# jean-pierreBoth/kmerutils

Measured on AMD Instinct MI355X. Metric: Gbases/sec k-mer+sketch throughput, k=31, 200 sketches/read, higher is better.
Workload: dtype u64; 1 GPU; ont_k31: 746333 ONT-shaped reads (log-normal lengths, 8% errors), 4.38e+09 bases, k=31, ProbMinHash3a m=200 + kmercount 8-bit; workload_name=ont_k31, reads_per_gpu=746333, bases_per_gpu=4379626696, kmers_per_gpu=4357236706, k=31, sketch_size=200, sketch=True, count=True, parallelism=reads sharded x1

## Files before the change

kmerutils_amd/csrc/kmu_pmh_points.hip:

```cpp
#include "kmu_pmh_steps.h"

namespace kmu {

static constexpr uint32_t PTS_REFRESH_MASK = 15u;

template <bool UNIT_W = false>
__device__ __forceinline__ bool pmh3a_first_point_may_matter(const SketchArgs &a, bool sig32, uint64_t qb, uint64_t key,
                                                             uint32_t w, const double *winv_lut, uint64_t &s0, uint64_t &s3) {
    const uint64_t seed = hasher_finish(KMU_HASHER_NOHASH, key, sig32);
    s0 = splitmix_at(seed, 1);
    s3 = splitmix_at(seed, 4);
    const uint64_t r1 = rotl64(s0 + s3, 23) + s0;
    const double u1 = __longlong_as_double((long long) ((r1 >> 12) | 0x3FF0000000000000ull)) - 1.0;
    const double x = a.e01.c1 * u1;
    if (UNIT_W) return !(x < 1.0) || x < __longlong_as_double((long long) qb);
    return !(x < 1.0) || winv_of(winv_lut, w) * x < __longlong_as_double((long long) qb);
}

__device__ __forceinline__ void pmh3a_first_point_rest(const SketchArgs &a, bool sig32, uint64_t *hmin, uint64_t *sig,
                                                       const uint64_t *qmax_sh, bool have, uint64_t key, uint32_t w,
                                                       uint64_t s0, uint64_t s3, const double *winv_lut) {
    const uint64_t qb = __hip_atomic_load(qmax_sh, __ATOMIC_RELAXED, __HIP_MEMORY_SCOPE_WORKGROUP);
    if (have) {
        const double winv = winv_of(winv_lut, w);
        const uint64_t r1 = rotl64(s0 + s3, 23) + s0;
        const double u1 = __longlong_as_double((long long) ((r1 >> 12) | 0x3FF0000000000000ull)) - 1.0;
        double x = a.e01.c1 * u1;
        const double qmax = __longlong_as_double((long long) qb);
        const bool slow = !(x < 1.0);
        if (slow || winv * x < qmax) {
            const uint64_t seed = hasher_finish(KMU_HASHER_NOHASH, key, sig32);
            Xoshiro rng;
            rng.s0 = s0;
            rng.s3 = s3;
            rng.s1 = splitmix_at(seed, 2);
            rng.s2 = splitmix_at(seed, 3);
            (void) rng.next();
            if (slow) x = exp01_rest(a.e01, rng);
            const double h = winv * x;
            if (h < qmax) slot_update_wave(hmin, sig, draw_slot(a, rng), h, key);
        }
    }
}

__global__ void __launch_bounds__(256) k_pts_long_list(const uint32_t *lst_n, uint32_t n_seq, uint32_t thr, uint32_t *out) {
    const uint32_t r = blockIdx.x * blockDim.x + threadIdx.x;
    if (r < n_seq && lst_n[r] > thr) out[2 + atomicAdd(&out[0], 1u)] = r;
}
__device__ __forceinline__ uint64_t wg4_qmax(const uint64_t *arrays, size_t wave_words, int m) {
    uint64_t q = 0;
    for (int t = lane_id(); t < m; t += 64) {
        uint64_t v = H_INIT;
#pragma unroll
        for (int w4 = 0; w4 < 4; w4++) {
            const uint64_t x = __hip_atomic_load(&arrays[(size_t) w4 * wave_words + t], __ATOMIC_RELAXED, __HIP_MEMORY_SCOPE_WORKGROUP);
            v = x < v ? x : v;
        }
        q = v > q ? v : q;
    }
    return wave_max_u64(q);
}

template <bool SIG32, bool WG>
__device__ __forceinline__ void pts_one_read(const SketchArgs &a, uint32_t r, uint8_t *smem, size_t wave_words, const double *winv_lut) {
    const int wave = threadIdx.x >> 6, lane = lane_id();
    constexpr bool sig32 = SIG32;
    constexpr uint32_t cstride = WG ? 256u : 64u;
    const uint32_t cstart = WG ? 64u * (uint32_t) wave : 0u;
    uint64_t *arrays = reinterpret_cast<uint64_t *>(smem);
    uint64_t *hmin = arrays + (size_t) wave * wave_words;
    uint64_t *sig = hmin + a.m;
    uint64_t *qmax_sh = sig + a.m;
    uint64_t *qk = qmax_sh + 2;
    uint32_t *qw = reinterpret_cast<uint32_t *>(qk + 128);
    uint64_t *qs0 = qk + 128 + 64, *qs3 = qs0 + 128;
    const uint64_t base = a.offsets[r] - a.offsets[0];
    const uint32_t n = uniform_u32(a.lst_n[r]);
    const uint32_t n_u = uniform_u32(a.lst_nu[r]);
    uint64_t tau_b = H_INIT;
    if (n >= a.tau_min_n) {
        const uint64_t len = a.offsets[r + 1] - a.offsets[r];
        const uint64_t kk = (uint64_t) a.cfg.k;
        const double tau = a.tau_num / (double) (len >= kk ? len - kk + 1 : 0);
        if (tau < 1.0) tau_b = (uint64_t) __double_as_longlong(tau);
        tau_b = uniform_u64(tau_b);
    }
    uint32_t wmax = 0;
    uint64_t qb = H_INIT;
    for (int turn = 0; turn < 2; turn++) {
        for (int t = lane; t < a.m; t += 64) { hmin[t] = H_INIT; sig[t] = 0; }
        if (lane == 0) *qmax_sh = tau_b;
        if (WG) __syncthreads();
        uint32_t chunk = 0, qn = 0;
        qb = tau_b;
        uint64_t key_nx = 0;
        uint32_t w_nx = 1;
        {
            const uint32_t i = cstart + (uint32_t) lane;
            if (i < n) { key_nx = a.lst_keys[base + i]; w_nx = i < n_u ? 1u : a.lst_w[base + i]; }
        }
        for (uint32_t c = cstart; c < n; c += cstride, chunk++) {
            const uint32_t i = c + (uint32_t) lane;
            const uint64_t key = key_nx;
            const uint32_t w = w_nx;
            const bool have = i < n && w != 0u;
            if (have) wmax = w > wmax ? w : wmax;
            if (i + cstride < n) key_nx = a.lst_keys[base + i + cstride];
            w_nx = 1u;
            if (c + cstride + 64u > n_u) {
                if (i + cstride < n && i + cstride >= n_u) w_nx = a.lst_w[base + i + cstride];
            }
            if ((chunk & (WG && chunk < 64u ? PTS_REFRESH_MASK >> 2 : PTS_REFRESH_MASK)) == 0u) {
                qb = WG ? wg4_qmax(arrays, wave_words, a.m) : wave_qmax(hmin, a.m);
                qb = qb < tau_b ? qb : tau_b;
                if (lane == 0) *qmax_sh = qb;
            }
            uint64_t s0 = 0, s3 = 0;
            const bool pass = c + 64u <= n_u ? have && pmh3a_first_point_may_matter<true>(a, sig32, qb, key, w, winv_lut, s0, s3)
                                             : have && pmh3a_first_point_may_matter(a, sig32, qb, key, w, winv_lut, s0, s3);
            const uint64_t pm = __ballot(pass);
            if (pass) {
                const uint32_t pos = qn + (uint32_t) __popcll(pm & ((1ull << lane) - 1ull));
                qk[pos] = key;
                qw[pos] = w;
                qs0[pos] = s0;
                qs3[pos] = s3;
            }
            qn += (uint32_t) __popcll(pm);
            if (qn >= 64u) {
                qn -= 64u;
                pmh3a_first_point_rest(a, sig32, hmin, sig, qmax_sh, true, qk[qn + lane], qw[qn + lane], qs0[qn + lane], qs3[qn + lane],
                                       winv_lut);
            }
        }
        if (qn) {
            const bool have = (uint32_t) lane < qn;
            pmh3a_first_point_rest(a, sig32, hmin, sig, qmax_sh, have, have ? qk[lane] : 0ull, have ? qw[lane] : 1u, have ? qs0[lane] : 0ull,
                                   have ? qs3[lane] : 0ull, winv_lut);
        }
        if (WG) {
            __syncthreads();
            qb = wg4_qmax(arrays, wave_words, a.m);
        } else qb = wave_qmax(hmin, a.m);
        if (tau_b == H_INIT || qb < tau_b) break;
        tau_b = H_INIT;
        if (lane == 0 && (!WG || wave == 0)) atomicAdd(a.tau_redo, 1u);
        if (WG) __syncthreads();
    }
    wmax = (uint32_t) wave_max_u64((uint64_t) wmax);
    if (n && wmax && winv_of(winv_lut, wmax) < __longlong_as_double((long long) qb)) {
        const uint32_t c0 = 1.0 < __longlong_as_double((long long) qb) ? 0u : (n_u & ~63u);
        uint32_t c = cstart;
        if (c < c0) c += (c0 - c + cstride - 1u) / cstride * cstride;
        for (; c < n; c += cstride) {
            const uint32_t i = c + (uint32_t) lane;
            double winv = 0.0;
            bool alive = false;
            if (i < n) {
                const uint32_t w = i < n_u ? 1u : a.lst_w[base + i];
                winv = winv_of(winv_lut, w);
                alive = w != 0u && winv < __longlong_as_double((long long) qb);
            }
            if (__any(alive)) pmh3a_more_points<true>(a, sig32, hmin, sig, qb, alive, alive ? a.lst_keys[base + i] : 0ull, winv);
        }
    }
    if (WG) {
        __syncthreads();
        for (int t = threadIdx.x; t < a.m; t += 256) {
            uint64_t bh = arrays[t], bk = arrays[a.m + t];
#pragma unroll
            for (int w4 = 1; w4 < 4; w4++) {
// ... 77 lines not shown
```

kmerutils_amd/csrc/kmu_api.hip:

```cpp
#include <algorithm>

#include "kmu_ctx.hpp"
#include "kmu_stream.h"

namespace kmu {

thread_local std::string g_create_error;

int check_kmer(kmu_ctx *ctx, int t, int k) {
    if (k <= 0) return fail(ctx, KMU_E_BAD_K, "kmer_size %d must be positive", k);
    int maxk = 0;
    switch (t) {
    case KMU_KMER32BIT: maxk = 14; break;
    case KMU_KMER16B32BIT:
        if (k != 16) return fail(ctx, KMU_E_BAD_K, "Kmer16b32bit has 16 bases, got %d", k);
        return KMU_OK;
    case KMU_KMER64BIT: maxk = 31; break;
    case KMU_KMERAA32BIT: maxk = 6; break;
    case KMU_KMERAA64BIT: maxk = 12; break;
    default: return fail(ctx, KMU_E_BAD_ARG, "unknown kmer_type %d", t);
    }
    if (k > maxk)
        return fail(ctx, KMU_E_BAD_K, "KmerSeqIterator cannot support so many bases for given kmer type, kmer size %d", k);
    return KMU_OK;
// ... 333 lines not shown
    KMU_HIP(ctx, hipStreamSynchronize(ctx->stream));
    KMU_HIP(ctx, hipHostFree(p));
    return KMU_OK;
}

int kmu_copy_to_device(kmu_ctx *ctx, void *dst_device, const void *src_host, uint64_t bytes) {
    if (!ctx || (bytes && (!dst_device || !src_host))) return KMU_E_BAD_ARG;
    KMU_HIP(ctx, hipSetDevice(ctx->device));
    KMU_HIP(ctx, hipMemcpyAsync(dst_device, src_host, bytes, hipMemcpyHostToDevice, ctx->stream));
    KMU_HIP(ctx, hipStreamSynchronize(ctx->stream));
    return KMU_OK;
}

int kmu_copy_to_host(kmu_ctx *ctx, void *dst_host, const void *src_device, uint64_t bytes) {
    if (!ctx || (bytes && (!dst_host || !src_device))) return KMU_E_BAD_ARG;
    KMU_HIP(ctx, hipSetDevice(ctx->device));
    KMU_HIP(ctx, hipMemcpyAsync(dst_host, src_device, bytes, hipMemcpyDeviceToHost, ctx->stream));
    KMU_HIP(ctx, hipStreamSynchronize(ctx->stream));
    return KMU_OK;
}

int kmu_profile_enable(kmu_ctx *ctx, int on) {
    if (!ctx) return KMU_E_BAD_ARG;
    if (!on && ctx->profiling) profile_collect(ctx);
    ctx->profiling = on != 0;
    return KMU_OK;
}
int kmu_profile_reset(kmu_ctx *ctx) {
    if (!ctx) return KMU_E_BAD_ARG;
    profile_collect(ctx);
    ctx->stats.clear();
    auto tr = ctx->bufs.find("pmh.tau_redo");
    if (tr != ctx->bufs.end() && tr->second.p) KMU_HIP(ctx, hipMemsetAsync(tr->second.p, 0, 4, ctx->stream));
    return KMU_OK;
}
int kmu_profile_get(kmu_ctx *ctx, kmu_kernel_stat *stats, int cap) {
    if (!ctx) return KMU_E_BAD_ARG;
    profile_collect(ctx);
    int n = 0;
    for (auto &kv : ctx->stats) {
        if (stats && n < cap) {
            memset(&stats[n], 0, sizeof(kmu_kernel_stat));
            strncpy(stats[n].name, kv.first.c_str(), sizeof(stats[n].name) - 1);
            stats[n].launches = kv.second.launches;
            stats[n].total_ms = kv.second.ms;
        }
        n++;
    }
    auto tr = ctx->bufs.find("pmh.tau_redo");
    if (tr != ctx->bufs.end() && tr->second.p) {
        uint32_t redone = 0;
        KMU_HIP(ctx, hipMemcpyAsync(&redone, tr->second.p, 4, hipMemcpyDeviceToHost, ctx->stream));
        KMU_HIP(ctx, hipStreamSynchronize(ctx->stream));
        if (redone) {
            if (stats && n < cap) {
                memset(&stats[n], 0, sizeof(kmu_kernel_stat));
                strncpy(stats[n].name, "pmh_tau_redone_reads", sizeof(stats[n].name) - 1);
                stats[n].launches = redone;
            }
            n++;
        }
    }
    return n;
}

int kmu_count_non_acgt(kmu_ctx *ctx, const uint8_t *bases, const uint64_t *offsets, uint32_t n_seq, int mem,
                       uint64_t *counts_out) {
    if (!ctx || !counts_out) return KMU_E_BAD_ARG;
    KMU_HIP(ctx, hipSetDevice(ctx->device));
    DevSeqs ds;
    KMU_TRY(stage_sequences(ctx, bases, offsets, nullptr, n_seq, KMU_INPUT_ASCII, mem, &ds));
    uint64_t *d_counts = counts_out;
    if (mem == KMU_MEM_HOST) {
        void *p;
        KMU_TRY(dev_buf(ctx, "out.u64", (size_t) n_seq * 8 + 8, &p));
        d_counts = (uint64_t *) p;
    }
    if (n_seq) {
        int grid = (int) std::min<uint32_t>(n_seq, (uint32_t) ctx->num_cus * 8);
        KernelTimer t(ctx, "k_count_non_acgt");
        hipLaunchKernelGGL(k_count_non_acgt, dim3(grid), dim3(256), 0, ctx->stream, ds.bases, ds.offsets, n_seq,
                           ds.total_bytes, d_counts);
    }
    KMU_HIP(ctx, hipGetLastError());
    if (mem == KMU_MEM_HOST)
        KMU_HIP(ctx, hipMemcpyAsync(counts_out, d_counts, (size_t) n_seq * 8, hipMemcpyDeviceToHost, ctx->stream));
    return finish_call(ctx, mem);
}

int kmu_pack2b(kmu_ctx *ctx, const uint8_t *bases, const uint64_t *offsets, uint32_t n_seq, int mem,
               uint8_t *packed_out, uint64_t *packed_offsets_out) {
// ... 100 lines not shown
```

kmerutils_amd/csrc/kmu_sketch_kernels.h:

```cpp
#pragma once

#include "kmu_ctx.hpp"
#include "kmu_device.h"

namespace kmu {

struct SketchArgs {
    const uint8_t *bases;
    const uint64_t *offsets;
    const uint64_t *packed_offsets;
    const uint64_t *block_rows;
    uint32_t n_seq;
    int packed;
    uint64_t total_bytes;
    KmerCfg cfg;
    int m;
    int hasher;
    int rand08;
    int sig_bytes;
    uint32_t block_size;
    uint32_t cap;
    uint32_t part_target;
    double inv_part_target;
    uint32_t tile_shift;
    uint64_t *scr_keys;
    uint32_t *scr_info;
    uint32_t *scr_w;
    uint32_t skip_longer;
    uint64_t *def_keys;
    int bk_shift;
    uint32_t bk_mask;
    uint32_t *tau_redo;
    double tau_num;
    uint32_t *counts_out;
    const void *hashed;
    int hashed_bytes;
// ... 13 lines not shown
    uint32_t idx_thresh;
    uint64_t idx_zone;
    uint32_t tau_min_n;
    Exp01 e01;
    void *sig_out;
    uint32_t *queue;
    uint32_t *err;
};

enum { M_READ = 0, M_NSCR = 1, M_NEXT = 2, M_DEF = 3, M_QMAX = 4 , M_FLAGS = 6 , M_WORDS = 8 };
static constexpr uint32_t DEF_CAP = 1u << 20;
static constexpr uint32_t DEF_PARTS = 32;
static constexpr uint32_t DEF_SEG = DEF_CAP / DEF_PARTS;
static constexpr uint32_t LONG_SEQ_KMERS = 1u << 18;
static constexpr int BUCKET_BITS = 12;
static constexpr uint32_t NBUCKETS = 1u << BUCKET_BITS;
static constexpr int QCHUNK = 4;
static constexpr int KREG = 10;
static constexpr uint32_t WINV_LUT = 256;
static constexpr size_t PTS_WAVE_WORDS = 2 + 128 + 64 + 256;
static constexpr double PTS_TAU_C = 4.6;
static constexpr int UQ_KREG = 20;
static constexpr uint32_t UQ1_BM = 17, UQ1_COLL = 1024, UQ2_BM = 18, UQ2_COLL = 2048;
template <int UQ_THREADS, uint32_t UQ_BM_BITS, uint32_t UQ_COLL>
struct UqShape {
    static constexpr uint32_t KEYS = (uint32_t) UQ_THREADS * UQ_KREG;
    static constexpr uint32_t BM_WORDS = (1u << UQ_BM_BITS) / 32;
    static constexpr uint32_t BUCKETS = 2u * UQ_THREADS;
    static constexpr uint32_t TILE = (KEYS + 32 + 15) / 16 + 3;
    static constexpr uint32_t RAW_WAVES = (TILE + 63) / 64;
    static constexpr size_t LDS = (size_t) BM_WORDS * 8 + (size_t) UQ_COLL * 20 + ((size_t) BUCKETS + 1 + TILE + UQ_THREADS / 64 + 8 + 8) * 4 + 64 +
                                  (size_t) RAW_WAVES * 1024 + 16;
};
static constexpr uint32_t SHORT_KEYS = 256, SHORT_SLOTS = 512, SHORT_WORDS = 24;
static constexpr size_t SHORT_WAVE_BYTES = (size_t) SHORT_SLOTS * 12 + SHORT_WORDS * 4;
static constexpr uint32_t SMALLK_WORDS = 32768;
static constexpr uint32_t SMALLK_TILE = 1024;

template <bool AA, bool BOTTOMK, bool EMIT = false, bool PLAIN = false>
__global__ void __launch_bounds__(1024) k_sketch_pmh3a(SketchArgs a);
__global__ void k_pts_long_list(const uint32_t *lst_n, uint32_t n_seq, uint32_t thr, uint32_t *out);
template <bool SIG32>
__global__ void __launch_bounds__(256) k_pmh_points(SketchArgs a);
template <int UQ_THREADS, uint32_t UQ_BM_BITS, uint32_t UQ_COLL, int MINW>
__global__ void __launch_bounds__(UQ_THREADS, MINW) k_multiset_uq(SketchArgs a);
__global__ void k_multiset_short(SketchArgs a);
template <bool SIG32>
__global__ void __launch_bounds__(256) k_pmh_points_short(SketchArgs a);
template <bool EMIT>
__global__ void __launch_bounds__(1024) k_sketch_smallk(SketchArgs a);
__global__ void k_pmh_reduce(const uint64_t *part_h, const uint64_t *part_k, uint64_t n_parts, int m, uint64_t stride, int sig_bytes, void *sig_out,
                             uint64_t *part_out);
__global__ void k_max_len(const uint64_t *offsets, uint32_t n_seq, uint64_t *out);
__global__ void k_nk_scan(const uint64_t *offsets, uint32_t n_seq, int k, uint64_t *koff, uint32_t *err);
__global__ void k_seq_hashes_compact(const uint8_t *bases, const uint64_t *offsets, const uint64_t *packed_offsets, uint32_t n_seq, int packed,
                                     uint64_t total, KmerCfg cfg, const uint64_t *koff, uint64_t *out, uint32_t *err, int spread);
__global__ void k_widen_u32(const uint32_t *in, uint64_t n, uint64_t *out);

#define KMU_PMH_GENERAL_FORMS(X)                                                                                                    \
    X(k_sketch_pmh3a<false, false>) X(k_sketch_pmh3a<false, false, true>) X(k_sketch_pmh3a<true, true>) X(k_sketch_pmh3a<true, false>) \
    X(k_sketch_pmh3a<false, true>) X(k_sketch_pmh3a<false, false, false, true>)
#define KMU_PMH_POINTS_FORMS(X) X(k_pmh_points<true>) X(k_pmh_points<false>)
#define KMU_PMH_SHORT_FORMS(X) X(k_pmh_points_short<true>) X(k_pmh_points_short<false>)
#define KMU_PMH_UQ_FORMS(X) X(k_multiset_uq<512, UQ1_BM, UQ1_COLL, 4>) X(k_multiset_uq<1024, UQ2_BM, UQ2_COLL, 4>)
#define KMU_PMH_SMALLK_FORMS(X) X(k_sketch_smallk<true>) X(k_sketch_smallk<false>)
#define KMU_SKETCH_KERNEL_FORMS(X) \
    KMU_PMH_GENERAL_FORMS(X) KMU_PMH_POINTS_FORMS(X) KMU_PMH_SHORT_FORMS(X) KMU_PMH_UQ_FORMS(X) KMU_PMH_SMALLK_FORMS(X)
#define KMU_X_EXTERN(...) extern template __global__ void __VA_ARGS__(SketchArgs);
KMU_SKETCH_KERNEL_FORMS(KMU_X_EXTERN)
#undef KMU_X_EXTERN

}
```

kmerutils_amd/csrc/kmu_sketch_pmh.hip:

```cpp
#include <algorithm>
#include <cmath>

#include "kmu_sketch_host.hpp"
#include "kmu_sketch_kernels.h"

using namespace kmu;

static int atoi_or(const char *s, int dflt) { return s ? atoi(s) : dflt; }

static bool smallk_route(const kmu_sketch_params *p, int hashed_bytes, bool partial, bool blocks) {
    if (p->algo != KMU_ALGO_PROB3A || p->kmer_type != KMU_KMER32BIT || p->kmer_size > 8 || hashed_bytes || partial || blocks ||
        p->block_size != 0 || p->sketch_size > 512)
        return false;
    switch (p->fhash) {
    case KMU_FHASH_IDENTITY_RAW: case KMU_FHASH_VALUE_MASKED: case KMU_FHASH_CANON_RAW: case KMU_FHASH_CANON_INVHASH:
    case KMU_FHASH_INVHASH_RAW: case KMU_FHASH_CANON_VALUE: break;
    default: return false;
    }
    return atoi_or(getenv("KMU_PMH_SMALLK"), 1) != 0;
}

enum class PmhRoute { SMALLK, SHORT, UQ, LISTS, ONE_PASS, GENERAL };
struct PmhPlan {
    PmhRoute route = PmhRoute::GENERAL;
    bool lists = false;
    uint64_t list_bases = 0;
    uint32_t pts_long = 32768;
    int cus = 0;
};

static int alloc_lists(kmu_ctx *ctx, SketchArgs &a, uint64_t bases) {
    void *lk, *lw, *ln;
    KMU_TRY(dev_buf(ctx, "cnt.partA", bases * 8 + 64, &lk));
    KMU_TRY(dev_buf(ctx, "pmh.lst_w", bases * 4 + 64, &lw));
    KMU_TRY(dev_buf(ctx, "pmh.lst_n", (size_t) a.n_seq * 8 + 64, &ln));
    a.lst_keys = (uint64_t *) lk;
    a.lst_w = (uint32_t *) lw;
    a.lst_n = (uint32_t *) ln;
    a.lst_nu = a.lst_n + a.n_seq;
    KMU_HIP(ctx, hipMemsetAsync(a.lst_nu, 0, (size_t) a.n_seq * 4, ctx->stream));
    return KMU_OK;
}

static int pmh_route(kmu_ctx *ctx, const kmu_sketch_params *p, const DevSeqs &ds, const PmhInputs &in, PmhPlan *plan) {
    const int split_mode = atoi_or(getenv("KMU_PMH_SPLIT"), -1);
    const bool plain_on = atoi_or(getenv("KMU_PMH_PLAIN"), 1) != 0;
    const bool short_on = atoi_or(getenv("KMU_PMH_SHORT"), 1) != 0;
    plan->pts_long = (uint32_t) std::max(0, atoi_or(getenv("KMU_PMH_PTS_LONG"), 32768));
    const int cus = ctx->num_cus;
    plan->cus = std::max(cus / 2, cus - std::max(0, atoi_or(getenv("KMU_PMH_RESERVE_CUS"), 0)));
    const bool smallk = smallk_route(p, in.hashed_bytes, in.part_h != nullptr, in.d_block_rows != nullptr);
    const bool whole = p->algo != KMU_ALGO_BOTTOMK && !kmer_is_aa(p->kmer_type) && !in.hashed_bytes && !in.part_h &&
                       !in.d_block_rows && p->block_size == 0;
    bool lists = (size_t) 4 * (2 * (size_t) p->sketch_size + PTS_WAVE_WORDS) * 8 + WINV_LUT * 8 <= 150 * 1024 &&
                 split_mode != 0 && (smallk || (whole && !in.skip_longer && (split_mode == 1 || in.len_stats)));
    const bool judge = !smallk && split_mode != 1;
    if (lists) {
        uint64_t &total = plan->list_bases;
        if (in.len_stats) total = in.len_stats[1];
        else if (!ds.h_offsets.empty()) total = ds.h_offsets[ds.n_seq] - ds.h_offsets[0];
        else {
            uint64_t ends[2] = {0, 0};
            KMU_HIP(ctx, hipMemcpyAsync(&ends[0], ds.offsets, 8, hipMemcpyDeviceToHost, ctx->stream));
            KMU_HIP(ctx, hipMemcpyAsync(&ends[1], ds.offsets + ds.n_seq, 8, hipMemcpyDeviceToHost, ctx->stream));
            KMU_HIP(ctx, hipStreamSynchronize(ctx->stream));
            total = ends[1] - ends[0];
        }
        if (judge) {
            const uint64_t longest = in.len_stats[0];
            const double cu_share = (double) ctx->num_cus / 256.0;
            const double wave_rate = plan->pts_long && longest > plan->pts_long ? 1.6e5 : 4.0e4;
            const double t_ideal = (double) total / (2.35e8 * cu_share), t_tail = (double) longest / wave_rate;
            const double overhang = t_tail >= t_ideal ? t_tail - 0.5 * t_ideal : t_tail * t_tail / (2.0 * t_ideal);
            const double gain = 0.43 * (double) total / (4.9e7 * cu_share);
            if (gain <= overhang + 0.02) lists = false;
        }
        if (lists && (smallk || judge)) {
            const size_t need_k = total * 8 + 64, need_w = total * 4 + 64;
            size_t grow = 0, free_b = 0, total_b = 0;
            if (ctx->bufs["cnt.partA"].bytes < need_k) grow += need_k + need_k / 8;
            if (ctx->bufs["pmh.lst_w"].bytes < need_w) grow += need_w + need_w / 8;
// ... 142 lines not shown
    a.read_list = a.redo_list;
    a.n_queue = n;
    return launch_main(ctx, a, kern, (int) std::min<uint64_t>((uint64_t) n, g.slots), g.lds, name);
}

static int read_count(kmu_ctx *ctx, const SketchArgs &a, uint32_t *n) {
    KMU_HIP(ctx, hipMemcpyAsync(n, a.queue + 56, 4, hipMemcpyDeviceToHost, ctx->stream));
    KMU_HIP(ctx, hipStreamSynchronize(ctx->stream));
    return KMU_OK;
}

static int launch_short(kmu_ctx *ctx, const SketchArgs &a, int cus) {
    const size_t lds_s = 4 * SHORT_WAVE_BYTES;
    const int per_cu = 5;
    {
        KernelTimer t(ctx, "k_multiset_short");
        hipLaunchKernelGGL(k_multiset_short, dim3((unsigned) std::max<uint64_t>(1, std::min<uint64_t>(((uint64_t) a.n_seq + 3) / 4, (uint64_t) cus * per_cu))),
                           dim3(256), lds_s, ctx->stream, a);
    }
    KMU_HIP(ctx, hipGetLastError());
    KMU_HIP(ctx, hipMemsetAsync(a.queue, 0, 256, ctx->stream));
    const sketch_kernel_t kpts = a.sig_bytes == 4 ? k_pmh_points_short<true> : k_pmh_points_short<false>;
    const size_t lds2 = (size_t) 4 * (2 * (size_t) a.m + 2) * 8 + WINV_LUT * 8;
    if (lds2 > 64 * 1024)
        KMU_HIP(ctx, hipFuncSetAttribute((const void *) kpts, hipFuncAttributeMaxDynamicSharedMemorySize, 160 * 1024));
    const int per_cu2 = (int) std::max<size_t>(1, std::min<size_t>(4, (160 * 1024) / lds2));
    const int grid2 = (int) std::max<uint64_t>(1, std::min<uint64_t>(((uint64_t) a.n_seq + 3) / 4, (uint64_t) cus * per_cu2));
    KernelTimer t(ctx, "k_pmh_points_short");
    hipLaunchKernelGGL(kpts, dim3(grid2), dim3(256), lds2, ctx->stream, a);
    KMU_HIP(ctx, hipGetLastError());
    return KMU_OK;
}

static int launch_uq(kmu_ctx *ctx, SketchArgs a, sketch_kernel_t kern, const PmhShape &g, const PmhPlan &plan) {
    {
        const auto ka = k_multiset_uq<512, UQ1_BM, UQ1_COLL, 4>;
        const size_t lds_a = UqShape<512, UQ1_BM, UQ1_COLL>::LDS;
        KMU_HIP(ctx, hipFuncSetAttribute((const void *) ka, hipFuncAttributeMaxDynamicSharedMemorySize, 80 * 1024));
        KernelTimer t(ctx, "k_multiset_uq");
        hipLaunchKernelGGL(ka, dim3((unsigned) std::max<uint64_t>(1, std::min<uint64_t>(a.n_seq, (uint64_t) plan.cus * 2))), dim3(512), lds_a,
                           ctx->stream, a);
    }
    KMU_HIP(ctx, hipGetLastError());
    uint32_t n_long = 0;
    KMU_TRY(read_count(ctx, a, &n_long));
    if (n_long) {
        const auto kb = k_multiset_uq<1024, UQ2_BM, UQ2_COLL, 4>;
        const size_t lds_b = UqShape<1024, UQ2_BM, UQ2_COLL>::LDS;
        void *rl2;
        KMU_TRY(dev_buf(ctx, "pmh.redo2", (size_t) a.n_seq * 4 + 64, &rl2));
        KMU_HIP(ctx, hipFuncSetAttribute((const void *) kb, hipFuncAttributeMaxDynamicSharedMemorySize, 160 * 1024));
        KMU_HIP(ctx, hipMemsetAsync(a.queue, 0, 256, ctx->stream));
        SketchArgs b = a;
        b.read_list = a.redo_list;
        b.redo_list = (uint32_t *) rl2;
        b.n_queue = n_long;
        {
            KernelTimer t(ctx, "k_multiset_uq");
            hipLaunchKernelGGL(kb, dim3((unsigned) std::max<uint64_t>(1, std::min<uint64_t>(n_long, (uint64_t) plan.cus))), dim3(1024), lds_b, ctx->stream, b);
        }
        KMU_HIP(ctx, hipGetLastError());
        KMU_TRY(read_count(ctx, a, &n_long));
        a.redo_list = b.redo_list;
    }
    if (n_long) KMU_TRY(launch_listed(ctx, a, kern, g, n_long, "k_sketch_pmh3a"));
    KMU_HIP(ctx, hipMemsetAsync(a.queue, 0, 256, ctx->stream));
    return launch_points(ctx, a, plan.cus, plan.pts_long);
}

static int launch_one_pass(kmu_ctx *ctx, const SketchArgs &a, sketch_kernel_t kern, const PmhShape &g) {
    KMU_TRY(launch_main(ctx, a, kern, g.grid, g.lds, "k_sketch_pmh3a"));
    uint32_t n_redo = 0;
    KMU_TRY(read_count(ctx, a, &n_redo));
    if (n_redo) KMU_TRY(launch_listed(ctx, a, k_sketch_pmh3a<false, false>, g, n_redo, "k_sketch_pmh3a_redo"));
    return KMU_OK;
}

static SketchArgs sketch_args(const kmu_sketch_params *p, const DevSeqs &ds, void *d_sig, uint32_t *d_err, const PmhInputs &in) {
    SketchArgs a;
    memset(&a, 0, sizeof a);
    a.skip_longer = in.skip_longer;
    a.hashed = in.hashed;
    a.hashed_bytes = in.hashed_bytes;
    a.part_h = in.part_h;
    a.part_k = in.part_k;
    a.bases = ds.bases;
    a.offsets = ds.offsets;
    a.packed_offsets = ds.packed_offsets;
    a.block_rows = in.d_block_rows;
    a.n_seq = ds.n_seq;
    a.n_queue = ds.n_seq;
    a.packed = ds.packed;
    a.total_bytes = ds.total_bytes;
    a.cfg = KmerCfg{p->kmer_type, in.hashed_bytes ? 1 : p->kmer_size, p->fhash};
    a.m = p->sketch_size;
    a.hasher = p->hasher;
// ... 115 lines not shown
```

Before: 49.97 Gbases/s.

## Process two key chunks per loop trip in PMH3a first-point filter

Unrolls the per-read key scan so each wave handles two 64-key chunks per trip, with double-buffered prefetch of keys and weights and an unconditional load fast path away from the tail. In the all-unit-weight region it skips the have/wmax checks and seeds wmax from n_u, and queue push/drain moves into helpers that use mbcnt for compaction. The qmax refresh mask is halved so the refresh cadence in elements stays the same. More live registers may reduce occupancy, and the wmax seeding changes the condition for the later second phase.

After: 50.14 Gbases/s (median of 6 runs). Within noise of the previous version (+0.4%).

```diff
diff --git a/kmerutils_amd/csrc/kmu_pmh_points.hip b/kmerutils_amd/csrc/kmu_pmh_points.hip
--- a/kmerutils_amd/csrc/kmu_pmh_points.hip
+++ b/kmerutils_amd/csrc/kmu_pmh_points.hip
@@ -2,7 +2,7 @@
 
 namespace kmu {
 
-static constexpr uint32_t PTS_REFRESH_MASK = 15u;
+static constexpr uint32_t PTS_REFRESH_MASK = 7u;
 
 template <bool UNIT_W = false>
 __device__ __forceinline__ bool pmh3a_first_point_may_matter(const SketchArgs &a, bool sig32, uint64_t qb, uint64_t key,
@@ -61,19 +61,52 @@
     return wave_max_u64(q);
 }
 
+struct PtsQueue {
+    uint64_t *k;
+    uint32_t *w;
+    uint64_t *s0, *s3;
+};
+__device__ __forceinline__ PtsQueue pts_queue_of(uint64_t *words) {
+    PtsQueue q;
+    q.k = words;
+    q.w = reinterpret_cast<uint32_t *>(words + 128);
+    q.s0 = words + 128 + 64;
+    q.s3 = q.s0 + 128;
+    return q;
+}
+__device__ __forceinline__ void pts_queue_push(const PtsQueue &q, uint32_t &qn, bool pass, uint64_t key, uint32_t w, uint64_t s0, uint64_t s3) {
+    const uint64_t pm = __ballot(pass);
+    if (pass) {
+        const uint32_t pos = __builtin_amdgcn_mbcnt_hi((uint32_t) (pm >> 32), __builtin_amdgcn_mbcnt_lo((uint32_t) pm, qn));
+        q.k[pos] = key;
+        q.w[pos] = w;
+        q.s0[pos] = s0;
+        q.s3[pos] = s3;
+    }
+    qn += (uint32_t) __popcll(pm);
+}
+__device__ __forceinline__ void pts_queue_work_off(const SketchArgs &a, bool sig32, uint64_t *hmin, uint64_t *sig, const uint64_t *qmax_sh,
+                                                   const PtsQueue &q, uint32_t &qn, const double *winv_lut) {
+    if (qn >= 64u) {
+        qn -= 64u;
+        const uint32_t e = qn + (uint32_t) lane_id();
+        pmh3a_first_point_rest(a, sig32, hmin, sig, qmax_sh, true, q.k[e], q.w[e], q.s0[e], q.s3[e], winv_lut);
+    }
+}
+
 template <bool SIG32, bool WG>
 __device__ __forceinline__ void pts_one_read(const SketchArgs &a, uint32_t r, uint8_t *smem, size_t wave_words, const double *winv_lut) {
     const int wave = threadIdx.x >> 6, lane = lane_id();
     constexpr bool sig32 = SIG32;
+    constexpr uint32_t tstride = WG ? 512u : 128u;
+    const uint32_t tstart = WG ? 128u * (uint32_t) wave : 0u;
     constexpr uint32_t cstride = WG ? 256u : 64u;
     const uint32_t cstart = WG ? 64u * (uint32_t) wave : 0u;
     uint64_t *arrays = reinterpret_cast<uint64_t *>(smem);
     uint64_t *hmin = arrays + (size_t) wave * wave_words;
     uint64_t *sig = hmin + a.m;
     uint64_t *qmax_sh = sig + a.m;
-    uint64_t *qk = qmax_sh + 2;
-    uint32_t *qw = reinterpret_cast<uint32_t *>(qk + 128);
-    uint64_t *qs0 = qk + 128 + 64, *qs3 = qs0 + 128;
+    const PtsQueue q = pts_queue_of(qmax_sh + 2);
     const uint64_t base = a.offsets[r] - a.offsets[0];
     const uint32_t n = uniform_u32(a.lst_n[r]);
     const uint32_t n_u = uniform_u32(a.lst_nu[r]);
@@ -85,58 +118,63 @@
         if (tau < 1.0) tau_b = (uint64_t) __double_as_longlong(tau);
         tau_b = uniform_u64(tau_b);
     }
-    uint32_t wmax = 0;
+    uint32_t wmax = n_u ? 1u : 0u;
     uint64_t qb = H_INIT;
     for (int turn = 0; turn < 2; turn++) {
         for (int t = lane; t < a.m; t += 64) { hmin[t] = H_INIT; sig[t] = 0; }
         if (lane == 0) *qmax_sh = tau_b;
         if (WG) __syncthreads();
-        uint32_t chunk = 0, qn = 0;
+        uint32_t trip = 0, qn = 0;
         qb = tau_b;
-        uint64_t key_nx = 0;
-        uint32_t w_nx = 1;
+        uint64_t key0_nx = 0, key1_nx = 0;
+        uint32_t w0_nx = 1, w1_nx = 1;
         {
-            const uint32_t i = cstart + (uint32_t) lane;
-            if (i < n) { key_nx = a.lst_keys[base + i]; w_nx = i < n_u ? 1u : a.lst_w[base + i]; }
-        }
-        for (uint32_t c = cstart; c < n; c += cstride, chunk++) {
-            const uint32_t i = c + (uint32_t) lane;
-            const uint64_t key = key_nx;
-            const uint32_t w = w_nx;
-            const bool have = i < n && w != 0u;
-            if (have) wmax = w > wmax ? w : wmax;
-            if (i + cstride < n) key_nx = a.lst_keys[base + i + cstride];
-            w_nx = 1u;
-            if (c + cstride + 64u > n_u) {
-                if (i + cstride < n && i + cstride >= n_u) w_nx = a.lst_w[base + i + cstride];
-            }
-            if ((chunk & (WG && chunk < 64u ? PTS_REFRESH_MASK >> 2 : PTS_REFRESH_MASK)) == 0u) {
+            const uint32_t i0 = tstart + (uint32_t) lane, i1 = i0 + 64u;
+            if (i0 < n) { key0_nx = a.lst_keys[base + i0]; w0_nx = i0 < n_u ? 1u : a.lst_w[base + i0]; }
+            if (i1 < n) { key1_nx = a.lst_keys[base + i1]; w1_nx = i1 < n_u ? 1u : a.lst_w[base + i1]; }
+        }
+        for (uint32_t c = tstart; c < n; c += tstride, trip++) {
+            const uint32_t i0 = c + (uint32_t) lane, i1 = i0 + 64u;
+            const uint64_t key0 = key0_nx, key1 = key1_nx;
+            const uint32_t w0 = w0_nx, w1 = w1_nx;
+            if (c + tstride + 128u <= n) {
+                key0_nx = a.lst_keys[base + i0 + tstride];
+                key1_nx = a.lst_keys[base + i1 + tstride];
+            } else {
+                if (i0 + tstride < n) key0_nx = a.lst_keys[base + i0 + tstride];
+                if (i1 + tstride < n) key1_nx = a.lst_keys[base + i1 + tstride];
+            }
+            w0_nx = w1_nx = 1u;
+            if (c + tstride + 128u > n_u) {
+                if (i0 + tstride < n && i0 + tstride >= n_u) w0_nx = a.lst_w[base + i0 + tstride];
+                if (i1 + tstride < n && i1 + tstride >= n_u) w1_nx = a.lst_w[base + i1 + tstride];
+            }
+            if ((trip & (WG && trip < 32u ? PTS_REFRESH_MASK >> 2 : PTS_REFRESH_MASK)) == 0u) {
                 qb = WG ? wg4_qmax(arrays, wave_words, a.m) : wave_qmax(hmin, a.m);
                 qb = qb < tau_b ? qb : tau_b;
                 if (lane == 0) *qmax_sh = qb;
             }
-            uint64_t s0 = 0, s3 = 0;
-            const bool pass = c + 64u <= n_u ? have && pmh3a_first_point_may_matter<true>(a, sig32, qb, key, w, winv_lut, s0, s3)
-                                             : have && pmh3a_first_point_may_matter(a, sig32, qb, key, w, winv_lut, s0, s3);
-            const uint64_t pm = __ballot(pass);
-            if (pass) {
-                const uint32_t pos = qn + (uint32_t) __popcll(pm & ((1ull << lane) - 1ull));
-                qk[pos] = key;
-                qw[pos] = w;
-                qs0[pos] = s0;
-                qs3[pos] = s3;
-            }
-            qn += (uint32_t) __popcll(pm);
-            if (qn >= 64u) {
-                qn -= 64u;
-                pmh3a_first_point_rest(a, sig32, hmin, sig, qmax_sh, true, qk[qn + lane], qw[qn + lane], qs0[qn + lane], qs3[qn + lane],
-                                       winv_lut);
-            }
+            uint64_t s0a = 0, s3a = 0, s0b = 0, s3b = 0;
+            bool pass0, pass1;
+            if (c + 128u <= n_u) {
+                pass0 = pmh3a_first_point_may_matter<true>(a, sig32, qb, key0, 1u, winv_lut, s0a, s3a);
+                pass1 = pmh3a_first_point_may_matter<true>(a, sig32, qb, key1, 1u, winv_lut, s0b, s3b);
+            } else {
+                const bool have0 = i0 < n && w0 != 0u, have1 = i1 < n && w1 != 0u;
+                if (have0) wmax = w0 > wmax ? w0 : wmax;
+                if (have1) wmax = w1 > wmax ? w1 : wmax;
+                pass0 = have0 && pmh3a_first_point_may_matter(a, sig32, qb, key0, w0, winv_lut, s0a, s3a);
+                pass1 = have1 && pmh3a_first_point_may_matter(a, sig32, qb, key1, w1, winv_lut, s0b, s3b);
+            }
+            pts_queue_push(q, qn, pass0, key0, w0, s0a, s3a);
+            pts_queue_work_off(a, sig32, hmin, sig, qmax_sh, q, qn, winv_lut);
+            pts_queue_push(q, qn, pass1, key1, w1, s0b, s3b);
+            pts_queue_work_off(a, sig32, hmin, sig, qmax_sh, q, qn, winv_lut);
         }
         if (qn) {
             const bool have = (uint32_t) lane < qn;
-            pmh3a_first_point_rest(a, sig32, hmin, sig, qmax_sh, have, have ? qk[lane] : 0ull, have ? qw[lane] : 1u, have ? qs0[lane] : 0ull,
-                                   have ? qs3[lane] : 0ull, winv_lut);
+            pmh3a_first_point_rest(a, sig32, hmin, sig, qmax_sh, have, have ? q.k[lane] : 0ull, have ? q.w[lane] : 1u, have ? q.s0[lane] : 0ull,
+                                   have ? q.s3[lane] : 0ull, winv_lut);
         }
         if (WG) {
             __syncthreads();
```

## Split long reads into segments for second-stage multiset dedup and merge

Applied to the files above, without the earlier changes.

Reads that overflow the first unique-kmer pass are now cut into fixed-size segments, each handled as its own item by the 1024-thread dedup kernel. A new merge kernel then combines duplicate keys across segments with an LDS bitmap and hash table, and hands back any read it cannot merge to the fallback sketch path. The goal is to balance work for very long ONT reads and send fewer reads to the slow k_sketch_pmh3a fallback. The cost is extra kernels, buffers and a device-to-host copy of the counters, and the added merge logic is complex and has give-up paths.

After: 49.78 Gbases/s before, 50.10 Gbases/s after (median of 6 runs). Within noise of the previous version (+0.6%).

```diff
diff --git a/kmerutils_amd/csrc/kmu_api.hip b/kmerutils_amd/csrc/kmu_api.hip
--- a/kmerutils_amd/csrc/kmu_api.hip
+++ b/kmerutils_amd/csrc/kmu_api.hip
@@ -389,6 +389,8 @@
     ctx->stats.clear();
     auto tr = ctx->bufs.find("pmh.tau_redo");
     if (tr != ctx->bufs.end() && tr->second.p) KMU_HIP(ctx, hipMemsetAsync(tr->second.p, 0, 4, ctx->stream));
+    auto sg = ctx->bufs.find("pmh.seg_stat");
+    if (sg != ctx->bufs.end() && sg->second.p) KMU_HIP(ctx, hipMemsetAsync(sg->second.p, 0, 8, ctx->stream));
     return KMU_OK;
 }
 int kmu_profile_get(kmu_ctx *ctx, kmu_kernel_stat *stats, int cap) {
@@ -414,6 +416,22 @@
                 memset(&stats[n], 0, sizeof(kmu_kernel_stat));
                 strncpy(stats[n].name, "pmh_tau_redone_reads", sizeof(stats[n].name) - 1);
                 stats[n].launches = redone;
+            }
+            n++;
+        }
+    }
+    auto sg = ctx->bufs.find("pmh.seg_stat");
+    if (sg != ctx->bufs.end() && sg->second.p) {
+        uint32_t seg[2] = {0, 0};
+        KMU_HIP(ctx, hipMemcpyAsync(seg, sg->second.p, 8, hipMemcpyDeviceToHost, ctx->stream));
+        KMU_HIP(ctx, hipStreamSynchronize(ctx->stream));
+        static const char *const names[2] = {"pmh_seg_reads", "pmh_seg_handed_back"};
+        for (int i = 0; i < 2; i++) {
+            if (!seg[i]) continue;
+            if (stats && n < cap) {
+                memset(&stats[n], 0, sizeof(kmu_kernel_stat));
+                strncpy(stats[n].name, names[i], sizeof(stats[n].name) - 1);
+                stats[n].launches = seg[i];
             }
             n++;
         }
diff --git a/kmerutils_amd/csrc/kmu_pmh_seg.hip b/kmerutils_amd/csrc/kmu_pmh_seg.hip
--- /dev/null
+++ b/kmerutils_amd/csrc/kmu_pmh_seg.hip
@@ -0,0 +1,179 @@
+#include "kmu_pmh_steps.h"
+
+namespace kmu {
+
+__global__ void __launch_bounds__(256) k_seg_plan(SegArgs a) {
+    const uint32_t i = blockIdx.x * blockDim.x + threadIdx.x;
+    if (i == 0) { a.so[0] = a.offsets[0]; a.so[1] = a.offsets[a.n_seq]; }
+    if (i >= *a.n_redo) return;
+    const uint32_t r = a.redo_in[i];
+    const uint64_t begin = a.offsets[r], nk = a.offsets[r + 1] - begin - (uint64_t) a.k + 1;
+    const SegSplit sp = seg_split(nk, a.balanced != 0);
+    const uint32_t first = atomicAdd(&a.cnt[SEG_CNT_SEGS], sp.nseg);
+    if (sp.nseg > 1) {
+        const uint32_t m = atomicAdd(&a.cnt[SEG_CNT_MULTI], 1u);
+        a.multi[2 * m] = r;
+        a.multi[2 * m + 1] = first;
+    }
+    for (uint32_t j = 0; j < sp.nseg; j++) {
+        const uint32_t s = first + j;
+        a.so[2 * (s + 1)] = begin + seg_first(sp, j);
+        a.so[2 * (s + 1) + 1] = begin + seg_end(sp, j, nk) + (uint64_t) a.k - 1;
+        a.seg_list[s] = 2 * (s + 1);
+        a.seg_read[s] = sp.nseg > 1 ? 0xFFFFFFFFu : r;
+    }
+}
+
+__device__ __forceinline__ uint32_t seg_fold(uint64_t key) { return (uint32_t) key ^ (uint32_t) (key >> 32); }
+
+__global__ void __launch_bounds__(1024) k_seg_merge(SegArgs a) {
+    constexpr uint32_t T = 1024, TSLOTS = 1u << SEG_TABLE_BITS, BM_WORDS = (1u << SEG_BM_BITS) / 32;
+    constexpr int KR = 40;
+    constexpr uint32_t CHUNK = KR * T;
+    constexpr uint64_t EMPTY = 0xFFFFFFFFFFFFFFFFull;
+    extern __shared__ __attribute__((aligned(16))) uint8_t smem[];
+    uint64_t *tkey = reinterpret_cast<uint64_t *>(smem);
+    uint32_t *tsum = reinterpret_cast<uint32_t *>(tkey + TSLOTS);
+    uint32_t *tmin = tsum + TSLOTS;
+    uint32_t *bm = reinterpret_cast<uint32_t *>(smem);
+    uint64_t *cand = reinterpret_cast<uint64_t *>(tmin + TSLOTS);
+    uint32_t *match = reinterpret_cast<uint32_t *>(cand);
+    uint32_t *misc = reinterpret_cast<uint32_t *>(cand + SEG_CAND);
+    uint32_t *sn = misc + 8, *snu = sn + SEG_MAX_SEGS;
+    const uint32_t tid = threadIdx.x;
+    const uint32_t n_segs = a.cnt[SEG_CNT_SEGS], n_multi = a.cnt[SEG_CNT_MULTI];
+    for (uint32_t s = blockIdx.x * T + tid; s < n_segs; s += gridDim.x * T) {
+        const uint32_t r = a.seg_read[s];
+        if (r == 0xFFFFFFFFu) continue;
+        const uint32_t n = a.seg_n[2 * (s + 1)];
+        a.lst_n[r] = n;
+        a.lst_nu[r] = n ? a.seg_nu[2 * (s + 1)] : 0u;
+        if (!n) { a.redo_out[atomicAdd(a.redo_cnt, 1u)] = r; atomicAdd(&a.stat[1], 1u); }
+    }
+    const uint64_t off_first = a.offsets[0];
+    for (;;) {
+        if (tid == 0) { misc[0] = atomicAdd(&a.cnt[SEG_CNT_CURSOR], 1u); misc[3] = 0; }
+        __syncthreads();
+        const uint32_t it = misc[0];
+        if (it >= n_multi) break;
+        const uint32_t r = a.multi[2 * it], first = a.multi[2 * it + 1];
+        const uint64_t begin = a.offsets[r], lb = begin - off_first;
+        const uint32_t nk = (uint32_t) (a.offsets[r + 1] - begin - (uint64_t) a.k + 1);
+        const SegSplit sp = seg_split(nk, a.balanced != 0);
+        if (tid < sp.nseg && tid < SEG_MAX_SEGS) {
+            sn[tid] = a.seg_n[2 * (first + tid + 1)];
+            snu[tid] = a.seg_nu[2 * (first + tid + 1)];
+            if (sn[tid] == 0) misc[3] = 1;
+        }
+        if (tid == 0 && sp.nseg > SEG_MAX_SEGS) misc[3] = 1;
+        __syncthreads();
+        bool give_up = misc[3] != 0;
+        const uint32_t parts = seg_merge_parts(nk), chunks = (nk + CHUNK - 1) / CHUNK;
+        uint64_t rk[KR];
+        uint64_t live = 0;
+        auto load_chunk = [&](uint32_t c, bool first_time) {
+            const uint32_t pos0 = c * CHUNK + tid;
+            uint32_t j = pos0 / sp.S, next = (j + 1) * sp.S;
+            live = 0;
+#pragma unroll
+            for (int e = 0; e < KR; e++) {
+                const uint32_t pos = pos0 + (uint32_t) e * T;
+                rk[e] = 0;
+                if (pos < nk) {
+                    if (pos >= next) { j++; next += sp.S; }
+                    const uint32_t ii = pos - (next - sp.S);
+                    if (ii < sn[j]) {
+                        const bool implied = ii < snu[j];
+                        const uint32_t w = implied ? 1u : a.lst_w[lb + pos];
+                        rk[e] = a.lst_keys[lb + pos];
+                        if (w) live |= 1ull << e;
+                        if (first_time && implied) a.lst_w[lb + pos] = 1u;
+                    } else if (first_time) a.lst_w[lb + pos] = 0u;
+                }
+            }
+        };
+        auto part_of = [&](uint32_t fold) -> uint32_t { return (uint32_t) (((uint64_t) (fold * 0xC2B2AE35u) * parts) >> 32); };
+        auto slot_of = [&](uint32_t fold) -> uint32_t { return (fold * 0x9E3779B1u) >> (32 - SEG_TABLE_BITS); };
+        for (uint32_t p = 0; p < parts && !give_up; p++) {
+            __syncthreads();
+            for (uint32_t t = tid; t < BM_WORDS / 4; t += T) reinterpret_cast<uint4 *>(bm)[t] = make_uint4(0u, 0u, 0u, 0u);
+            if (tid == 0) { misc[1] = 0; misc[2] = 0; }
+            __syncthreads();
+            for (uint32_t c = 0; c < chunks; c++) {
+                if (chunks > 1 || p == 0) load_chunk(c, p == 0);
+#pragma unroll
+                for (int e = 0; e < KR; e++) {
+                    if (!((live >> e) & 1ull)) continue;
+                    const uint32_t fold = seg_fold(rk[e]);
+                    if (parts > 1 && part_of(fold) != p) continue;
+                    const uint32_t bi = (fold * 0x85EBCA6Bu) >> (32 - SEG_BM_BITS), bit = 1u << (bi & 31u);
+                    if (atomicOr(&bm[bi >> 5], bit) & bit) {
+                        const uint32_t ci = atomicAdd(&misc[1], 1u);
+                        if (ci < SEG_CAND) cand[ci] = rk[e];
+                    }
+                }
+            }
+            __syncthreads();
+            const uint32_t nc = misc[1];
+            if (nc > SEG_CAND) { give_up = true; break; }
+            if (nc == 0) continue;
+            uint64_t ck[SEG_CAND / T];
+#pragma unroll
+            for (uint32_t u = 0; u < SEG_CAND / T; u++) ck[u] = tid + u * T < nc ? cand[tid + u * T] : 0ull;
+            for (uint32_t t = tid; t < TSLOTS; t += T) { tkey[t] = EMPTY; tsum[t] = 0u; tmin[t] = 0xFFFFFFFFu; }
+            __syncthreads();
+#pragma unroll
+            for (uint32_t u = 0; u < SEG_CAND / T; u++) {
+                if (tid + u * T >= nc) continue;
+                if (ck[u] == EMPTY) { misc[3] = 1; continue; }
+                for (uint32_t s = slot_of(seg_fold(ck[u]));; s = (s + 1) & (TSLOTS - 1)) {
+                    const uint64_t old = atomicCAS((unsigned long long *) &tkey[s], (unsigned long long) EMPTY, (unsigned long long) ck[u]);
+                    if (old == EMPTY || old == ck[u]) break;
+                }
+            }
+            __syncthreads();
+            if (misc[3]) { give_up = true; break; }
+            for (uint32_t c = 0; c < chunks; c++) {
+                if (chunks > 1) load_chunk(c, false);
+#pragma unroll
+                for (int e = 0; e < KR; e++) {
+                    if (!((live >> e) & 1ull)) continue;
+                    const uint64_t key = rk[e];
+                    const uint32_t fold = seg_fold(key);
+                    if (parts > 1 && part_of(fold) != p) continue;
+                    uint32_t s = slot_of(fold);
+                    for (;; s = (s + 1) & (TSLOTS - 1)) {
+                        const uint64_t t = tkey[s];
+                        if (t == key) break;
+                        if (t == EMPTY) { s = TSLOTS; break; }
+                    }
+                    if (s == TSLOTS) continue;
+                    const uint32_t pos = c * CHUNK + tid + (uint32_t) e * T, j = pos / sp.S;
+                    const uint32_t w = pos - j * sp.S < snu[j] ? 1u : a.lst_w[lb + pos];
+                    atomicAdd(&tsum[s], w);
+                    atomicMin(&tmin[s], pos);
+                    const uint32_t mi = atomicAdd(&misc[2], 1u);
+                    if (mi < SEG_MATCH) match[mi] = (s << 19) | pos;
+                }
+            }
+            __syncthreads();
+            const uint32_t nm = misc[2];
+            if (nm > SEG_MATCH) { give_up = true; break; }
+            for (uint32_t t = tid; t < nm; t += T) {
+                const uint32_t s = match[t] >> 19, pos = match[t] & 0x7FFFFu;
+                a.lst_w[lb + pos] = tmin[s] == pos ? tsum[s] : 0u;
+            }
+        }
+        if (tid == 0) {
+            atomicAdd(&a.stat[0], 1u);
+            if (give_up) {
+                a.lst_n[r] = 0u;
+                a.redo_out[atomicAdd(a.redo_cnt, 1u)] = r;
+                atomicAdd(&a.stat[1], 1u);
+            } else a.lst_n[r] = nk;
+        }
+        __syncthreads();
+    }
+}
+
+}
diff --git a/kmerutils_amd/csrc/kmu_seg_plan.hpp b/kmerutils_amd/csrc/kmu_seg_plan.hpp
--- /dev/null
+++ b/kmerutils_amd/csrc/kmu_seg_plan.hpp
@@ -0,0 +1,27 @@
+#pragma once
+
+#include <stdint.h>
+
+namespace kmu {
+
+static constexpr uint32_t SEG_S_MAX = 1024u * 20u - 16u;
+
+struct SegSplit { uint32_t nseg, S; };
+constexpr SegSplit seg_split(uint64_t nk, bool balanced) {
+    const uint32_t nseg = (uint32_t) ((nk + SEG_S_MAX - 1) / SEG_S_MAX);
+    return SegSplit{nseg, nseg <= 1 ? SEG_S_MAX : balanced ? (uint32_t) ((nk + nseg - 1) / nseg) : SEG_S_MAX};
+}
+constexpr uint64_t seg_first(SegSplit s, uint32_t j) { return (uint64_t) j * s.S; }
+constexpr uint64_t seg_end(SegSplit s, uint32_t j, uint64_t nk) { return (uint64_t) (j + 1) * s.S < nk ? (uint64_t) (j + 1) * s.S : nk; }
+
+constexpr uint64_t seg_bound(uint64_t n_redo, uint64_t total_bases) { return n_redo + total_bases / SEG_S_MAX; }
+
+static constexpr uint32_t SEG_BM_BITS = 19, SEG_PART_KEYS = 1u << 15, SEG_CAND = 3072, SEG_TABLE_BITS = 13, SEG_MATCH = 2 * SEG_CAND;
+static constexpr uint32_t SEG_MAX_SEGS = 16;
+constexpr uint32_t seg_merge_parts(uint64_t nk) { return (uint32_t) ((nk + SEG_PART_KEYS - 1) / SEG_PART_KEYS); }
+static constexpr uint32_t SEG_MERGE_LDS = (1u << SEG_TABLE_BITS) * 16u + SEG_CAND * 8u + 256u;
+static_assert((1u << SEG_BM_BITS) / 8u <= (1u << SEG_TABLE_BITS) * 16u, "the bitmap lies inside the table's space");
+static_assert(SEG_MATCH * 4u <= SEG_CAND * 8u, "the matched entries lie inside the candidates' space");
+static_assert(SEG_MERGE_LDS <= 160u * 1024u, "one workgroup's LDS");
+
+}
diff --git a/kmerutils_amd/csrc/kmu_sketch_kernels.h b/kmerutils_amd/csrc/kmu_sketch_kernels.h
--- a/kmerutils_amd/csrc/kmu_sketch_kernels.h
+++ b/kmerutils_amd/csrc/kmu_sketch_kernels.h
@@ -2,6 +2,7 @@
 
 #include "kmu_ctx.hpp"
 #include "kmu_device.h"
+#include "kmu_seg_plan.hpp"
 
 namespace kmu {
 
@@ -81,6 +82,27 @@
     static constexpr size_t LDS = (size_t) BM_WORDS * 8 + (size_t) UQ_COLL * 20 + ((size_t) BUCKETS + 1 + TILE + UQ_THREADS / 64 + 8 + 8) * 4 + 64 +
                                   (size_t) RAW_WAVES * 1024 + 16;
 };
+static_assert(SEG_S_MAX == UqShape<1024, UQ2_BM, UQ2_COLL>::KEYS - 16, "a segment fits the second shape whatever its first base's place");
+enum { SEG_CNT_SEGS = 0, SEG_CNT_MULTI = 1, SEG_CNT_CURSOR = 2, SEG_CNT_WORDS = 4 };
+struct SegArgs {
+    const uint64_t *offsets;
+    uint32_t n_seq;
+    int k;
+    int balanced;
+    const uint32_t *redo_in;
+    const uint32_t *n_redo;
+    uint64_t *so;
+    uint32_t *seg_list;
+    uint32_t *seg_read;
+    uint32_t *multi;
+    uint32_t *cnt;
+    const uint32_t *seg_n, *seg_nu;
+    uint64_t *lst_keys;
+    uint32_t *lst_w, *lst_n, *lst_nu;
+    uint32_t *redo_out;
+    uint32_t *redo_cnt;
+    uint32_t *stat;
+};
 static constexpr uint32_t SHORT_KEYS = 256, SHORT_SLOTS = 512, SHORT_WORDS = 24;
 static constexpr size_t SHORT_WAVE_BYTES = (size_t) SHORT_SLOTS * 12 + SHORT_WORDS * 4;
 static constexpr uint32_t SMALLK_WORDS = 32768;
@@ -93,6 +115,8 @@
 __global__ void __launch_bounds__(256) k_pmh_points(SketchArgs a);
 template <int UQ_THREADS, uint32_t UQ_BM_BITS, uint32_t UQ_COLL, int MINW>
 __global__ void __launch_bounds__(UQ_THREADS, MINW) k_multiset_uq(SketchArgs a);
+__global__ void __launch_bounds__(256) k_seg_plan(SegArgs a);
+__global__ void __launch_bounds__(1024) k_seg_merge(SegArgs a);
 __global__ void k_multiset_short(SketchArgs a);
 template <bool SIG32>
 __global__ void __launch_bounds__(256) k_pmh_points_short(SketchArgs a);
diff --git a/kmerutils_amd/csrc/kmu_sketch_pmh.hip b/kmerutils_amd/csrc/kmu_sketch_pmh.hip
--- a/kmerutils_amd/csrc/kmu_sketch_pmh.hip
+++ b/kmerutils_amd/csrc/kmu_sketch_pmh.hip
@@ -27,6 +27,7 @@
     uint64_t list_bases = 0;
     uint32_t pts_long = 32768;
     int cus = 0;
+    int seg = 1;
 };
 
 static int alloc_lists(kmu_ctx *ctx, SketchArgs &a, uint64_t bases) {
@@ -47,6 +48,7 @@
     const bool plain_on = atoi_or(getenv("KMU_PMH_PLAIN"), 1) != 0;
     const bool short_on = atoi_or(getenv("KMU_PMH_SHORT"), 1) != 0;
     plan->pts_long = (uint32_t) std::max(0, atoi_or(getenv("KMU_PMH_PTS_LONG"), 32768));
+    plan->seg = atoi_or(getenv("KMU_PMH_SEG"), 1);
     const int cus = ctx->num_cus;
     plan->cus = std::max(cus / 2, cus - std::max(0, atoi_or(getenv("KMU_PMH_RESERVE_CUS"), 0)));
     const bool smallk = smallk_route(p, in.hashed_bytes, in.part_h != nullptr, in.d_block_rows != nullptr);
@@ -255,7 +257,58 @@
     return KMU_OK;
 }
 
+static int seg_stat_buf(kmu_ctx *ctx, uint32_t **out) {
+    const bool fresh = !ctx->bufs.count("pmh.seg_stat");
+    void *st;
+    KMU_TRY(dev_buf(ctx, "pmh.seg_stat", 8, &st));
+    if (fresh) KMU_HIP(ctx, hipMemsetAsync(st, 0, 8, ctx->stream));
+    *out = (uint32_t *) st;
+    return KMU_OK;
+}
+
 static int launch_uq(kmu_ctx *ctx, SketchArgs a, sketch_kernel_t kern, const PmhShape &g, const PmhPlan &plan) {
+    const auto kb = k_multiset_uq<1024, UQ2_BM, UQ2_COLL, 4>;
+    const size_t lds_b = UqShape<1024, UQ2_BM, UQ2_COLL>::LDS;
+    SegArgs sg;
+    memset(&sg, 0, sizeof sg);
+    uint32_t *seg_queue = nullptr, *seg_redo = nullptr, *seg_counts = nullptr;
+    if (plan.seg) {
+        const uint64_t cap = seg_bound(a.n_seq, plan.list_bases);
+        void *so, *sl, *sr, *mu, *cn, *sc, *sq, *rd;
+        KMU_TRY(dev_buf(ctx, "seg.offsets", (cap + 1) * 16, &so));
+        KMU_TRY(dev_buf(ctx, "seg.list", cap * 4 + 64, &sl));
+        KMU_TRY(dev_buf(ctx, "seg.read", cap * 4 + 64, &sr));
+        KMU_TRY(dev_buf(ctx, "seg.multi", (size_t) a.n_seq * 8 + 64, &mu));
+        KMU_TRY(dev_buf(ctx, "seg.cnt", SEG_CNT_WORDS * 4, &cn));
+        KMU_TRY(dev_buf(ctx, "seg.lst_n", (cap + 1) * 16, &sc));
+        KMU_TRY(dev_buf(ctx, "seg.queue", 256, &sq));
+        KMU_TRY(dev_buf(ctx, "seg.redo", cap * 4 + 64, &rd));
+        KMU_HIP(ctx, hipMemsetAsync(cn, 0, SEG_CNT_WORDS * 4, ctx->stream));
+        KMU_HIP(ctx, hipMemsetAsync(sq, 0, 256, ctx->stream));
+        seg_queue = (uint32_t *) sq;
+        seg_redo = (uint32_t *) rd;
+        seg_counts = (uint32_t *) sc;
+        sg.offsets = a.offsets;
+        sg.n_seq = a.n_seq;
+        sg.k = a.cfg.k;
+        sg.balanced = plan.seg != 2;
+        sg.redo_in = a.redo_list;
+        sg.n_redo = a.queue + 56;
+        sg.so = (uint64_t *) so;
+        sg.seg_list = (uint32_t *) sl;
+        sg.seg_read = (uint32_t *) sr;
+        sg.multi = (uint32_t *) mu;
+        sg.cnt = (uint32_t *) cn;
+        sg.seg_n = seg_counts;
+        sg.seg_nu = seg_counts + 2 * (cap + 1);
+        sg.lst_keys = a.lst_keys;
+        sg.lst_w = a.lst_w;
+        sg.lst_n = a.lst_n;
+        sg.lst_nu = a.lst_nu;
+        KMU_TRY(seg_stat_buf(ctx, &sg.stat));
+    }
+    void *rl2;
+    KMU_TRY(dev_buf(ctx, "pmh.redo2", (size_t) a.n_seq * 4 + 64, &rl2));
     {
         const auto ka = k_multiset_uq<512, UQ1_BM, UQ1_COLL, 4>;
         const size_t lds_a = UqShape<512, UQ1_BM, UQ1_COLL>::LDS;
@@ -263,28 +316,42 @@
         KernelTimer t(ctx, "k_multiset_uq");
         hipLaunchKernelGGL(ka, dim3((unsigned) std::max<uint64_t>(1, std::min<uint64_t>(a.n_seq, (uint64_t) plan.cus * 2))), dim3(512), lds_a,
                            ctx->stream, a);
+        if (plan.seg) hipLaunchKernelGGL(k_seg_plan, dim3((a.n_seq + 255) / 256), dim3(256), 0, ctx->stream, sg);
     }
     KMU_HIP(ctx, hipGetLastError());
-    uint32_t n_long = 0;
+    uint32_t n_long = 0, h_cnt[SEG_CNT_WORDS] = {0, 0, 0, 0};
+    if (plan.seg) KMU_HIP(ctx, hipMemcpyAsync(h_cnt, sg.cnt, sizeof h_cnt, hipMemcpyDeviceToHost, ctx->stream));
     KMU_TRY(read_count(ctx, a, &n_long));
     if (n_long) {
-        const auto kb = k_multiset_uq<1024, UQ2_BM, UQ2_COLL, 4>;
-        const size_t lds_b = UqShape<1024, UQ2_BM, UQ2_COLL>::LDS;
-        void *rl2;
-        KMU_TRY(dev_buf(ctx, "pmh.redo2", (size_t) a.n_seq * 4 + 64, &rl2));
         KMU_HIP(ctx, hipFuncSetAttribute((const void *) kb, hipFuncAttributeMaxDynamicSharedMemorySize, 160 * 1024));
         KMU_HIP(ctx, hipMemsetAsync(a.queue, 0, 256, ctx->stream));
         SketchArgs b = a;
         b.read_list = a.redo_list;
         b.redo_list = (uint32_t *) rl2;
         b.n_queue = n_long;
+        if (plan.seg) {
+            b.offsets = sg.so;
+            b.n_seq = 1;
+            b.read_list = sg.seg_list;
+            b.n_queue = h_cnt[SEG_CNT_SEGS];
+            b.lst_n = seg_counts;
+            b.lst_nu = const_cast<uint32_t *>(sg.seg_nu);
+            b.queue = seg_queue;
+            b.redo_list = seg_redo;
+            sg.redo_out = (uint32_t *) rl2;
+            sg.redo_cnt = a.queue + 56;
+            KMU_HIP(ctx, hipFuncSetAttribute((const void *) k_seg_merge, hipFuncAttributeMaxDynamicSharedMemorySize, 160 * 1024));
+        }
         {
             KernelTimer t(ctx, "k_multiset_uq");
-            hipLaunchKernelGGL(kb, dim3((unsigned) std::max<uint64_t>(1, std::min<uint64_t>(n_long, (uint64_t) plan.cus))), dim3(1024), lds_b, ctx->stream, b);
+            hipLaunchKernelGGL(kb, dim3((unsigned) std::max<uint64_t>(1, std::min<uint64_t>(b.n_queue, (uint64_t) plan.cus))), dim3(1024), lds_b, ctx->stream, b);
+            if (plan.seg)
+                hipLaunchKernelGGL(k_seg_merge, dim3((unsigned) std::max<uint64_t>(1, std::min<uint64_t>(h_cnt[SEG_CNT_MULTI], (uint64_t) plan.cus))),
+                                   dim3(1024), SEG_MERGE_LDS, ctx->stream, sg);
         }
         KMU_HIP(ctx, hipGetLastError());
         KMU_TRY(read_count(ctx, a, &n_long));
-        a.redo_list = b.redo_list;
+        a.redo_list = (uint32_t *) rl2;
     }
     if (n_long) KMU_TRY(launch_listed(ctx, a, kern, g, n_long, "k_sketch_pmh3a"));
     KMU_HIP(ctx, hipMemsetAsync(a.queue, 0, 256, ctx->stream));
```
